# hobincar/reconstruction-network-for-video-captioning

Measured on NVIDIA B200. Metric: train samples/s (decoder+local rec fwd+bwd), higher is better.
Workload: dtype bf16

## Files before the change

reconstruction-network-for-video-captioning_b200/csrc/seq_decoder_cluster.cuh:

```cuda
#pragma once
#include <stdio.h>

#include "proj_attn.cuh"

namespace dcl {
constexpr int CS = 16;
constexpr int THREADS = 512;
constexpr int NWARP = THREADS / 32;
constexpr int MAX_MS = 16;
constexpr int MT = 16;
constexpr int H_ = 512, A_ = 128, UPC = 32, APC = 8, NR = APC + 4 * UPC;
constexpr int NRP = 144;
constexpr int PITCH = H_ + 8;
constexpr int MAXF = 2;
constexpr int MAXT = 32;

__device__ __forceinline__ uint32_t cta_rank() { uint32_t r; asm volatile("mov.u32 %0, %%cluster_ctarank;" : "=r"(r)); return r; }
__device__ __forceinline__ uint32_t cluster_id() { uint32_t r; asm volatile("mov.u32 %0, %%clusterid.x;" : "=r"(r)); return r; }
__device__ __forceinline__ void cluster_barrier() {
  asm volatile("barrier.cluster.arrive.release.aligned;" ::: "memory");
  asm volatile("barrier.cluster.wait.acquire.aligned;" ::: "memory");
}
__device__ __forceinline__ void cluster_arrive() { asm volatile("barrier.cluster.arrive.release.aligned;" ::: "memory"); }
__device__ __forceinline__ void cluster_wait() { asm volatile("barrier.cluster.wait.acquire.aligned;" ::: "memory"); }
__device__ __forceinline__ uint32_t smem_addr(const void* p) { return (uint32_t)__cvta_generic_to_shared(p); }
__device__ __forceinline__ uint32_t mapa(uint32_t saddr, uint32_t rank) {
  uint32_t r;
  asm volatile("mapa.shared::cluster.u32 %0, %1, %2;" : "=r"(r) : "r"(saddr), "r"(rank));
  return r;
}
__device__ __forceinline__ void st_c_f32(uint32_t a, float v) { asm volatile("st.shared::cluster.f32 [%0], %1;" ::"r"(a), "f"(v) : "memory"); }
__device__ __forceinline__ void st_c_f32x2(uint32_t a, float x, float y) { asm volatile("st.shared::cluster.v2.f32 [%0], {%1, %2};" ::"r"(a), "f"(x), "f"(y) : "memory"); }
__device__ __forceinline__ void st_c_f32x4(uint32_t a, float4 v) {
  asm volatile("st.shared::cluster.v4.f32 [%0], {%1, %2, %3, %4};" ::"r"(a), "f"(v.x), "f"(v.y), "f"(v.z), "f"(v.w) : "memory");
}
__device__ __forceinline__ void st_c_u32x4(uint32_t a, uint4 v) {
  asm volatile("st.shared::cluster.v4.b32 [%0], {%1, %2, %3, %4};" ::"r"(a), "r"(v.x), "r"(v.y), "r"(v.z), "r"(v.w) : "memory");
}
__device__ __forceinline__ void stamp(int tag) {
  if (g_timeline != nullptr && blockIdx.x == 0 && threadIdx.x == 0) {
    unsigned long long t;
    asm volatile("mov.u64 %0, %%globaltimer;" : "=l"(t));
    const unsigned int i = atomicAdd(&g_timeline_n, 1u);
    if (i < 4000) g_timeline[i] = (t & 0x00FFFFFFFFFFFFFFull) | ((unsigned long long)tag << 56);
  }
}
__device__ __forceinline__ void ldsm_x4(uint32_t (&r)[4], uint32_t addr) {
  asm volatile("ldmatrix.sync.aligned.m8n8.x4.shared.b16 {%0, %1, %2, %3}, [%4];" : "=r"(r[0]), "=r"(r[1]), "=r"(r[2]), "=r"(r[3]) : "r"(addr));
}
__device__ __forceinline__ void ldsm_x2(uint32_t (&r)[2], uint32_t addr) {
  asm volatile("ldmatrix.sync.aligned.m8n8.x2.shared.b16 {%0, %1}, [%2];" : "=r"(r[0]), "=r"(r[1]) : "r"(addr));
}
__device__ __forceinline__ void ldsm_x2_t(uint32_t (&r)[2], uint32_t addr) {
  asm volatile("ldmatrix.sync.aligned.m8n8.x2.trans.shared.b16 {%0, %1}, [%2];" : "=r"(r[0]), "=r"(r[1]) : "r"(addr));
}
__device__ __forceinline__ void mma16816(float (&c)[4], const uint32_t (&a)[4], const uint32_t (&b)[2]) {
  asm volatile("mma.sync.aligned.m16n8k16.row.col.f32.bf16.bf16.f32 {%0, %1, %2, %3}, {%4, %5, %6, %7}, {%8, %9}, {%0, %1, %2, %3};"
               : "+f"(c[0]), "+f"(c[1]), "+f"(c[2]), "+f"(c[3])
               : "r"(a[0]), "r"(a[1]), "r"(a[2]), "r"(a[3]), "r"(b[0]), "r"(b[1]));
}

__device__ __forceinline__ int wcat_row(int lr, int r) {
  return lr < APC ? r * APC + lr : A_ + ((lr - APC) / UPC) * H_ + r * UPC + (lr - APC) % UPC;
}

struct FwdArgs {
  const bf16* Wcat;
  const float* Uv;
  const float* attn_w;
  const bf16* VW;
  const float* Gx;
  const float* b_hh;
  float* c;
  float* hiddens;
  bf16* Hop;
  float* Wh; float* e;
  bf16* gates;
  int B, L, Tn, MS;
  float inv_T;
};

struct SmemF { int Ws, hs, og, whs, uvs, es, hst, part, total; };
__host__ __device__ inline SmemF smem_fwd() {
  SmemF s;
  s.Ws = 0;
  s.hs = s.Ws + NR * PITCH * 2;
  s.og = s.hs + MT * PITCH * 2;
  s.whs = s.og + MT * NR * 4;
  s.uvs = s.whs + MT * A_ * 4;
  s.es = s.uvs + MAXF * MT * A_ * 4;
  s.hst = s.es + MT * MAXT * 4;
  s.part = s.hst + NWARP * 32 * 2;
  s.total = s.part + NWARP * MT * APC * 4 + 16;
  return s;
}

template <int NQ, bool SM>
__global__ void __launch_bounds__(THREADS, 1) decoder_fwd_cluster_kernel(const FwdArgs a) {
  extern __shared__ __align__(16) unsigned char smem[];
  const SmemF S = smem_fwd();
  bf16* Ws = reinterpret_cast<bf16*>(smem + S.Ws);
  bf16* hs = reinterpret_cast<bf16*>(smem + S.hs);
  float* og = reinterpret_cast<float*>(smem + S.og);
  float* whs = reinterpret_cast<float*>(smem + S.whs);
  float* uvs = reinterpret_cast<float*>(smem + S.uvs);
  float* es = reinterpret_cast<float*>(smem + S.es);
  bf16* hst = reinterpret_cast<bf16*>(smem + S.hst);
  float* part = reinterpret_cast<float*>(smem + S.part);
  const int r = (int)cta_rank(), q = (int)cluster_id();
  const int tid = threadIdx.x, lane = tid & 31, warp = tid >> 5;
  const int B = a.B, Tn = a.Tn;
  const int b0 = q * a.MS, nb = min(a.MS, B - b0);
  if (nb <= 0) return;

  for (int i = tid; i < NR * (H_ / 8); i += THREADS) {
    const int lr = i / (H_ / 8), c8 = i - lr * (H_ / 8);
    *reinterpret_cast<uint4*>(Ws + (size_t)lr * PITCH + 8 * c8) = *reinterpret_cast<const uint4*>(a.Wcat + (size_t)wcat_row(lr, r) * H_ + 8 * c8);
  }
  for (int i = tid; i < MT * PITCH / 2; i += THREADS) reinterpret_cast<uint32_t*>(hs)[i] = 0u;
  for (int i = tid; i < MAXF * MT * (A_ / 4); i += THREADS) {
    const int f = i / (MT * (A_ / 4)), rem = i - f * (MT * (A_ / 4)), s = rem / (A_ / 4), c4 = rem - s * (A_ / 4);
    const int tau = r + CS * f;
    float4 v = make_float4(0.f, 0.f, 0.f, 0.f);
    if (tau < Tn && s < nb) v = reinterpret_cast<const float4*>(a.Uv + ((size_t)(b0 + s) * Tn + tau) * A_)[c4];
    reinterpret_cast<float4*>(uvs)[i] = v;
  }
  for (int i = tid; i < MT * MAXT; i += THREADS) es[i] = 0.f;
  for (int i = tid; i < MT * A_; i += THREADS) whs[i] = 0.f;
  for (int i = tid; i < MT * NR; i += THREADS) og[i] = 0.f;
  const bool act = warp < nb;
  const int s_w = min(warp, nb - 1), b = b0 + s_w;
  const int j = r * UPC + lane;
  pf::Quad<bf16> v[NQ];
  {
    const bf16* vw = a.VW + ((size_t)b * Tn * H_ + j) * 4;
#pragma unroll
    for (int k = 0; k < NQ; ++k) v[k].load(vw + (size_t)min(k, Tn - 1) * 4 * H_);
  }
  float bh[4];
#pragma unroll
  for (int g = 0; g < 4; ++g) bh[g] = a.b_hh[g * H_ + j];
  const float4 aw4 = reinterpret_cast<const float4*>(a.attn_w)[lane];
  float cstate = 0.f;
  __syncthreads();
  cluster_barrier();

  const uint32_t whs_sa = smem_addr(whs), es_sa = smem_addr(es), hs_sa = smem_addr(hs);
  const int gid = lane >> 2, tig = lane & 3;
  for (int t = 0; t < a.L; ++t) {
    float gx[4];
    {
      const float* gp = a.Gx + ((size_t)t * B + b) * 4 * H_ + j;
#pragma unroll
      for (int g = 0; g < 4; ++g) gx[g] = gp[g * H_];
    }
    stamp(20);
    if (t > 0) {
      cluster_wait();
      const uint32_t a_addr = hs_sa + (uint32_t)(((lane & 15) * PITCH + (lane >> 4) * 8) * 2);
      const uint32_t w_addr = smem_addr(Ws) + (uint32_t)(((lane & 7) * PITCH + ((lane >> 3) & 1) * 8) * 2);
      {
        float acc[4] = {0.f, 0.f, 0.f, 0.f};
#pragma unroll
        for (int kk = 0; kk < 2; ++kk) {
          uint32_t af[4], bfr[2];
          ldsm_x4(af, a_addr + (32 * warp + 16 * kk) * 2);
          ldsm_x2(bfr, w_addr + (32 * warp + 16 * kk) * 2);
          mma16816(acc, af, bfr);
        }
        float* pw = part + warp * (MT * APC);
        *reinterpret_cast<float2*>(pw + gid * APC + 2 * tig) = make_float2(acc[0], acc[1]);
        *reinterpret_cast<float2*>(pw + (gid + 8) * APC + 2 * tig) = make_float2(acc[2], acc[3]);
      }
      __syncthreads();
      {
        const int item = tid & 127, grp = tid >> 7, s_ = item >> 3, c_ = item & 7;
        float sum = 0.f;
#pragma unroll
        for (int w2 = 0; w2 < NWARP; ++w2) sum += part[w2 * (MT * APC) + item];
        const uint32_t dst_off = whs_sa + (uint32_t)((s_ * A_ + r * APC + c_) * 4);
#pragma unroll
        for (int i = 0; i < 4; ++i) st_c_f32(mapa(dst_off, (uint32_t)(grp * 4 + i)), sum);
      }
      stamp(27);
      cluster_arrive();
      {
        float acc0[4] = {0.f, 0.f, 0.f, 0.f}, acc1[4] = {0.f, 0.f, 0.f, 0.f};
        const uint32_t b_addr = w_addr + (uint32_t)((APC + warp * 8) * PITCH * 2);
#pragma unroll 2
        for (int k0 = 0; k0 < H_; k0 += 32) {
          uint32_t af[4], bfr[2], af2[4], bfr2[2];
          ldsm_x4(af, a_addr + k0 * 2);
          ldsm_x2(bfr, b_addr + k0 * 2);
          ldsm_x4(af2, a_addr + (k0 + 16) * 2);
          ldsm_x2(bfr2, b_addr + (k0 + 16) * 2);
          mma16816(acc0, af, bfr);
          mma16816(acc1, af2, bfr2);
        }
        const int n = APC + warp * 8 + 2 * tig;
        *reinterpret_cast<float2*>(og + gid * NR + n) = make_float2(acc0[0] + acc1[0], acc0[1] + acc1[1]);
        *reinterpret_cast<float2*>(og + (gid + 8) * NR + n) = make_float2(acc0[2] + acc1[2], acc0[3] + acc1[3]);
      }
      stamp(21);
      cluster_wait();
      stamp(22);
    }
    {
      const float4 wh = reinterpret_cast<const float4*>(whs + s_w * A_)[lane];
      if (r == 0 && act) reinterpret_cast<float4*>(a.Wh + ((size_t)t * B + b) * A_)[lane] = wh;
      float sc[MAXF];
#pragma unroll
      for (int f = 0; f < MAXF; ++f) {
        const float4 u = reinterpret_cast<const float4*>(uvs + (f * MT + s_w) * A_)[lane];
        float s = aw4.x * act_tanh<true>(wh.x + u.x);
        s = fmaf(aw4.y, act_tanh<true>(wh.y + u.y), s);
        s = fmaf(aw4.z, act_tanh<true>(wh.z + u.z), s);
        sc[f] = fmaf(aw4.w, act_tanh<true>(wh.w + u.w), s);
      }
#pragma unroll
      for (int o = 16; o > 0; o >>= 1)
#pragma unroll
        for (int f = 0; f < MAXF; ++f) sc[f] += __shfl_xor_sync(0xffffffffu, sc[f], o);
      const int f = lane & 1, tau = r + CS * f;
      const float val = f ? sc[1] : sc[0];
      if (act && tau < Tn) {
        st_c_f32(mapa(es_sa + (uint32_t)((s_w * MAXT + tau) * 4), (uint32_t)(lane >> 1)), val);
        if (!SM && lane < 2) a.e[((size_t)t * B + b) * Tn + tau] = val;
      }
    }
    stamp(23);
    cluster_barrier();
    stamp(24);
    if constexpr (SM) {
      float* er = es + s_w * MAXT;
      const float al = warp_softmax<true>(er[lane], lane < Tn);
      __syncwarp();
      if (act) {
        if (lane < Tn) er[lane] = al;
        if (r == 0 && lane < Tn) a.e[((size_t)t * B + b) * Tn + lane] = al;
      }
      __syncwarp();
    }
    {
      float acc[4] = {0.f, 0.f, 0.f, 0.f};
      const float4* e4 = reinterpret_cast<const float4*>(es + s_w * MAXT);
#pragma unroll
      for (int k4 = 0; k4 < NQ / 4; ++k4) {
        const float4 e = e4[k4];
        const float ev[4] = {e.x, e.y, e.z, e.w};
#pragma unroll
        for (int kk = 0; kk < 4; ++kk) {
          float f[4];
          v[4 * k4 + kk].get(f);
#pragma unroll
          for (int g = 0; g < 4; ++g) acc[g] = fmaf(ev[kk], f[g], acc[g]);
        }
      }
      float pre[4];
#pragma unroll
      for (int g = 0; g < 4; ++g) pre[g] = gx[g] + bh[g] + og[s_w * NR + APC + g * UPC + lane] + acc[g] * a.inv_T;
      const float gi = act_sigmoid<true>(pre[0]), gf = act_sigmoid<true>(pre[1]), gt = act_tanh<true>(pre[2]), go = act_sigmoid<true>(pre[3]);
      const float cn = fmaf(gf, cstate, gi * gt);
      const float hn = go * act_tanh<true>(cn);
      const bf16 hb = __float2bfloat16_rn(hn);
      hst[warp * 32 + lane] = hb;
      __syncwarp();
      if (act) {
#pragma unroll
        for (int i = 0; i < 2; ++i) {
          const int item = lane * 2 + i, dst = item >> 2, chunk = item & 3;
          const uint4 val = *reinterpret_cast<const uint4*>(hst + warp * 32 + chunk * 8);
          st_c_u32x4(mapa(hs_sa + (uint32_t)((s_w * PITCH + r * UPC + chunk * 8) * 2), (uint32_t)dst), val);
        }
      }
      cluster_arrive();
      if (act) {
        cstate = cn;
        const size_t o1 = ((size_t)t * B + b) * H_ + j;
        a.c[o1 + (size_t)B * H_] = cn;
        a.hiddens[o1] = hn;
        a.Hop[o1 + (size_t)B * H_] = hb;
        pf::Quad<bf16>::store(a.gates + o1 * 4, gi, gf, gt, go);
      }
    }
    stamp(25);
  }
  cluster_wait();
}

static inline bool cluster_enabled() {
  static const int v = rn_env_int("RECNET_DEC_CLUSTER", 1);
  return v != 0;
}
static inline bool cluster_ok(int B, int Tn, int A, int H) {
  return cluster_enabled() && H == H_ && A == A_ && Tn >= 1 && Tn <= MAXT && B >= 1 && B <= 8 * MAX_MS;
}

template <typename K>
static int launch_cluster(K kern, size_t smem, int B, cudaStream_t st, const void* args_struct_ptr, bool* configured) {
  (void)args_struct_ptr;
  if (!*configured) {
    if (cudaFuncSetAttribute(kern, cudaFuncAttributeNonPortableClusterSizeAllowed, 1) != cudaSuccess) { cudaGetLastError(); return RECNET_ERR_UNSUPPORTED; }
    if (cudaFuncSetAttribute(kern, cudaFuncAttributeMaxDynamicSharedMemorySize, (int)smem) != cudaSuccess) { cudaGetLastError(); return RECNET_ERR_UNSUPPORTED; }
    *configured = true;
  }
  return 0;
}

template <typename K>
static int pick_ms(K kern, size_t smem, int B) {
  cudaLaunchConfig_t cfg = {};
  cfg.gridDim = dim3(8 * CS, 1, 1);
  cfg.blockDim = dim3(THREADS, 1, 1);
  cfg.dynamicSmemBytes = smem;
  cudaLaunchAttribute at[1];
  at[0].id = cudaLaunchAttributeClusterDimension;
  at[0].val.clusterDim.x = CS; at[0].val.clusterDim.y = 1; at[0].val.clusterDim.z = 1;
  cfg.attrs = at; cfg.numAttrs = 1;
  int n = 0;
  if (cudaOccupancyMaxActiveClusters(&n, kern, &cfg) != cudaSuccess) { cudaGetLastError(); return 0; }
  n = rn_env_int("RECNET_DEC_CLUSTERS", n);
  if (rn_env_int("RECNET_DEBUG_CLUSTERS", 0)) fprintf(stderr, "[recnet] decoder cluster kernel: max active %d-CTA clusters = %d\n", CS, n);
  if (n < 1) return 0;
  const int ms = (B + n - 1) / n;
  return ms <= MAX_MS ? ms : 0;
}

template <int NQ, bool SM>
static int launch_fwd_nq(FwdArgs a, cudaStream_t st) {
  auto kern = decoder_fwd_cluster_kernel<NQ, SM>;
  const size_t smem = smem_fwd().total;
  static bool configured = false;
  static int ms_cache_B = -1, ms_cache = 0;
  RN_TRY(launch_cluster(kern, smem, a.B, st, nullptr, &configured));
  if (ms_cache_B != a.B) { ms_cache = pick_ms(kern, smem, a.B); ms_cache_B = a.B; }
  if (ms_cache <= 0) return RECNET_ERR_UNSUPPORTED;
  a.MS = ms_cache;
  const int ncl = (a.B + a.MS - 1) / a.MS;
  cudaLaunchConfig_t cfg = {};
  cfg.gridDim = dim3(ncl * CS, 1, 1);
  cfg.blockDim = dim3(THREADS, 1, 1);
  cfg.dynamicSmemBytes = smem;
  cfg.stream = st;
  cudaLaunchAttribute at[1];
  at[0].id = cudaLaunchAttributeClusterDimension;
  at[0].val.clusterDim.x = CS; at[0].val.clusterDim.y = 1; at[0].val.clusterDim.z = 1;
  cfg.attrs = at; cfg.numAttrs = 1;
  ProfScope prof(KC_LOOP, a.L, ncl * CS, 2, st);
  RN_CUDA_OK(cudaLaunchKernelEx(&cfg, kern, a));
  RN_LAUNCH_OK();
  return 0;
}
static int launch_fwd(const FwdArgs& a, bool softmax, cudaStream_t st) {
  if (softmax) return a.Tn <= 28 ? launch_fwd_nq<28, true>(a, st) : launch_fwd_nq<32, true>(a, st);
  return a.Tn <= 28 ? launch_fwd_nq<28, false>(a, st) : launch_fwd_nq<32, false>(a, st);
}
}
```

reconstruction-network-for-video-captioning_b200/csrc/seq_decoder_pf.cuh:

```cuda
#pragma once
#include "proj_attn.cuh"
#include "seq_decoder.cuh"
#include "seq_decoder_cluster.cuh"

namespace dec {

template <typename T>
struct PfWs {
  int EMBp, Vp, Vld, NP;
  GemmPlan pl_h, pl_dh;
  T *Wemb, *WctxI, *Wcat, *U, *Wout, *feats;
  float* Uv; T* VW; T* Xe; float* Gx; T* Hop; float* P; float* Wh; float* e; T* gates; float* c;
  float *logits, *lse, *row_loss;
  T* dlogits; float* dHext; T* dGW; float* dhP; float* dWh; float* dUv; T* dUv_op; float* dw_acc; float* dc; float* dXe; T* ctx;
  float* splitk; float* splitk2; float* splitk3; int* err;
  size_t bytes;
};

static inline bool pf_enabled() {
  static const int v = rn_env_int("RECNET_PF", 1);
  return v != 0;
}
static inline bool pf_ok(const recnet_decoder_desc& d) {
  if (!pf_enabled() || d.cell != RECNET_CELL_LSTM || d.n_layers > 1) return false;
  const int al = d.precision == RECNET_PREC_BF16 ? 8 : 4;
  if ((long long)d.B * d.T * 4 * d.H >= (1ll << 31) || (long long)d.L * d.B * (d.A + 4 * d.H) >= (1ll << 31)) return false;
  if ((d.E & 1) || pf::escore_smem(d.L, d.T, true) > 46 * 1024) return false;
  return d.T >= 1 && d.T <= pf::MAX_T && d.A >= 4 && d.A <= pf::MAX_A && d.A % al == 0 && d.H % al == 0 &&
         pf::bwd_smem_bytes(d.H, d.A) <= 46 * 1024;
}
enum class DecPath { ML, PF, GENERAL };
static inline DecPath dec_path(const recnet_decoder_desc& d) {
  if (d.n_layers > 1) return DecPath::ML;
  return pf_ok(d) ? DecPath::PF : DecPath::GENERAL;
}

template <typename T>
static PfWs<T> plan_pf(const recnet_decoder_desc& d, void* base) {
  PfWs<T> w;
  const int B = d.B, L = d.L, H = d.H, E = d.E, A = d.A, V = d.V, Tn = d.T;
  w.EMBp = round_up(d.EMB, Prec<T>::kpad);
  w.Vp = round_up(V, 8);
  w.Vld = round_up(V, 4);
  w.NP = A + 4 * H;
  w.pl_h = plan_gemm<T>(B, w.NP, H);
  w.pl_dh = plan_gemm<T>(B, H, w.NP);
  if (Prec<T>::id == RECNET_PREC_BF16) {
    w.pl_h.bn = 64;
    const int tiles = rn_cdiv(B, tc::BM) * rn_cdiv(w.NP, 64), nkb = rn_cdiv(H, tc::BK);
    int sp = NUM_SMS / tiles; if (sp < 1) sp = 1; if (sp > nkb) sp = nkb;
    w.pl_h.splits = rn_cdiv(nkb, rn_cdiv(nkb, sp));
    const int nkb2 = rn_cdiv(w.NP, tc::BK);
    if (w.pl_dh.splits > pf::MAXS) w.pl_dh.splits = rn_cdiv(nkb2, rn_cdiv(nkb2, pf::MAXS));
    static const int eh = rn_env_int("RECNET_PF_SPLITS_H", 0);
    static const int edh = rn_env_int("RECNET_PF_SPLITS_DH", 0);
    static const int ebn = rn_env_int("RECNET_PF_BN_H", 0);
    if (ebn == 64 || ebn == 128) w.pl_h.bn = ebn;
    if (eh > 0) w.pl_h.splits = rn_cdiv(nkb, rn_cdiv(nkb, eh > nkb ? nkb : eh));
    if (edh > 0) w.pl_dh.splits = rn_cdiv(nkb2, rn_cdiv(nkb2, edh > nkb2 ? nkb2 : edh));
  }
  Bump m(base);
  w.Wemb = m.take<T>((size_t)4 * H * w.EMBp);
  w.WctxI = m.take<T>((size_t)4 * H * E);
  w.Wcat = m.take<T>((size_t)w.NP * H);
  w.U = m.take<T>((size_t)A * E);
  w.Wout = m.take<T>((size_t)V * H);
  w.feats = m.take<T>((size_t)B * Tn * E);
  w.Uv = m.take<float>((size_t)B * Tn * A);
  w.VW = m.take<T>((size_t)B * Tn * 4 * H);
  w.Xe = m.take<T>((size_t)L * B * w.EMBp);
  w.Gx = m.take<float>((size_t)L * B * 4 * H);
  w.Hop = m.take<T>((size_t)(L + 1) * B * H);
  w.P = m.take<float>((size_t)w.pl_h.splits * B * w.NP);
  w.Wh = m.take<float>((size_t)L * B * A);
  w.e = m.take<float>((size_t)L * B * Tn);
  w.gates = m.take<T>((size_t)L * B * 4 * H);
  w.c = m.take<float>((size_t)(L + 1) * B * H);
  w.logits = m.take<float>((size_t)L * B * w.Vld);
  w.lse = m.take<float>((size_t)L * B);
  w.row_loss = m.take<float>((size_t)L * B);
  w.dlogits = m.take<T>((size_t)L * B * w.Vp);
  w.dHext = m.take<float>((size_t)L * B * H);
  w.dGW = m.take<T>((size_t)L * B * w.NP);
  w.dhP = m.take<float>((size_t)w.pl_dh.splits * B * H);
  w.dWh = m.take<float>((size_t)L * B * A);
  w.dUv = m.take<float>((size_t)B * Tn * A);
  w.dUv_op = m.take<T>((size_t)B * Tn * A);
  w.dw_acc = m.take<float>((size_t)B * A);
  w.dc = m.take<float>((size_t)B * H);
  w.dXe = m.take<float>((size_t)L * B * w.EMBp);
  w.ctx = m.take<T>((size_t)L * B * E);
  w.splitk = m.take<float>(SPLITK_SCRATCH_FLOATS);
  w.splitk2 = m.take<float>(SPLITK_SCRATCH_FLOATS);
  w.splitk3 = m.take<float>(SPLITK_SCRATCH_FLOATS);
  w.err = m.take<int>(64);
  w.bytes = m.off + 256;
  return w;
}

static inline int gemm_to_operand(const float* A, long long lda, const float* B, long long ldb, float* C, long long ldc, int M,
                                  int N, int K, float* scratch, cudaStream_t st) {
  return gemm_full<float>(A, lda, 0, B, ldb, 0, C, ldc, nullptr, M, N, K, 0, scratch, st);
}
static inline int gemm_to_operand(const bf16* A, long long lda, const bf16* B, long long ldb, bf16* C, long long ldc, int M, int N,
                                  int K, float*, cudaStream_t st) {
  GemmPlan p = plan_gemm_full<bf16>(M, N, K);
  if (p.splits > 1) p = plan_gemm<bf16>(M, N, K);
  return tc::launch(A, lda, 0, B, ldb, 0, nullptr, 0, C, ldc, nullptr, M, N, K, 1, 0, 0, p.bn, st);
}

template <typename T>
static int forward_pf(const DecDesc& d, const recnet_decoder_tensors& p, const float* feats, const long long* tokens_in,
                      const long long* targets, const float* ce_weight, const unsigned long long* rng, void* ws, long long ws_bytes,
                      float* hiddens, float* ce_out, cudaStream_t st, int phases = 3) {
  RN_TRY(check(d));
  PfWs<T> w = plan_pf<T>(d, ws);
  if ((long long)w.bytes > ws_bytes) return RECNET_ERR_WORKSPACE;
  const int B = d.B, L = d.L, H = d.H, E = d.E, A = d.A, V = d.V, Tn = d.T, EMB = d.EMB;
  const float p_emb = d.train ? d.p_emb_drop : 0.f, p_out = d.train ? d.p_out_drop : 0.f;
  const float inv_T = d.softmax ? 1.f : 1.f / Tn;
  const long long ldih = EMB + E;
  if (phases & 1) {
  cudaStream_t s2;
  RN_TRY(side().fork(st, &s2));
  misc::embed_gather_kernel<T><<<L * B, 128, 0, s2>>>(p.embedding, tokens_in, w.Xe, w.EMBp, L * B, EMB, w.EMBp, V, d.embedding_scale,
                                                      p_emb, rng, SITE_EMB);
  RN_LAUNCH_OK();
  misc::Stager<T> sg;
  sg.add(feats, E, w.feats, E, (long long)B * Tn, E, E);
  sg.add(p.attn_U, E, w.U, E, A, E, E);
  sg.add(p.w_ih, ldih, w.Wemb, w.EMBp, 4 * H, EMB, w.EMBp);
  sg.add(p.w_ih + EMB, ldih, w.WctxI, E, 4 * H, E, E, H);
  sg.add(p.attn_W, H, w.Wcat, H, A, H, H);
  sg.add(p.w_hh, H, w.Wcat + (size_t)A * H, H, 4 * H, H, H);
  sg.add(p.out_w, H, w.Wout, H, V, H, H);
  sg.zero(w.Hop, (size_t)B * H * sizeof(T));
  sg.zero(w.c, (size_t)B * H * sizeof(float));
  sg.zero(w.err, 64 * sizeof(int));
  RN_TRY(sg.launch(st));
  RN_TRY(side().fork(st, &s2));
  RN_TRY(gemm_full<T>(w.feats, E, 0, w.U, E, 0, w.Uv, A, p.attn_b, B * Tn, A, E, 0, w.splitk2, s2));
  RN_TRY(gemm_full<T>(w.Xe, w.EMBp, 0, w.Wemb, w.EMBp, 0, w.Gx, 4 * H, p.b_ih, L * B, 4 * H, w.EMBp, 0, w.splitk2, s2));
  RN_TRY(gemm_to_operand(w.feats, E, w.WctxI, E, w.VW, 4 * H, B * Tn, 4 * H, E, w.splitk, st));
  RN_TRY(side().join(st, s2));
  bool clustered = false;
  if constexpr (std::is_same<T, bf16>::value) {
    if (dcl::cluster_ok(B, Tn, A, H)) {
      dcl::FwdArgs ca{};
      ca.Wcat = w.Wcat; ca.Uv = w.Uv; ca.attn_w = p.attn_w; ca.VW = w.VW; ca.Gx = w.Gx; ca.b_hh = p.b_hh; ca.c = w.c; ca.hiddens = hiddens;
      ca.Hop = w.Hop; ca.Wh = w.Wh; ca.e = w.e; ca.gates = w.gates; ca.B = B; ca.L = L; ca.Tn = Tn; ca.inv_T = inv_T;
      const int rc = dcl::launch_fwd(ca, d.softmax, st);
      if (rc == 0) clustered = true;
      else if (rc != RECNET_ERR_UNSUPPORTED) return rc;
    }
  }
  for (int t = 0; t < L && !clustered; ++t) {
    const size_t r = (size_t)t * B;
    if (t > 0)
      RN_TRY(gemm_partials<T>(w.Hop + r * H, H, 0, w.Wcat, H, 0, w.P, B, w.NP, H, w.pl_h, st));
    pf::FwdArgs fa{};
    fa.P = w.P; fa.n_p = t > 0 ? w.pl_h.splits : 0; fa.p_stride = (long long)B * w.NP; fa.NP = w.NP;
    fa.Uv = w.Uv; fa.attn_w = p.attn_w; fa.VW = w.VW;
    fa.Gx = w.Gx + r * 4 * H; fa.b_hh = p.b_hh; fa.c_prev = w.c + r * H;
    fa.B = B; fa.Tn = Tn; fa.A = A; fa.H = H; fa.inv_T = inv_T;
    fa.Wh_out = w.Wh + r * A; fa.e_out = w.e + r * Tn; fa.gates_out = w.gates + r * 4 * H;
    fa.c_out = w.c + (r + B) * H; fa.h_out = hiddens + r * H; fa.h_op = w.Hop + (r + B) * H;
    RN_TRY((pf::launch_fwd<T, T>(fa, d.softmax, st)));
  }
  }
  if (!(phases & 2)) return 0;
  const bool training = targets && ce_weight && ce_out;
  cudaStream_t s3 = st;
  if (training) RN_TRY(side().fork(st, &s3));
  RN_TRY(gemm_full<T>(w.Hop + (size_t)B * H, H, 0, w.Wout, H, 0, w.logits, w.Vld, p.out_b, L * B, V, H, 0, w.splitk, st));
  if (training) {
    const int spc = 1;
    pf::pf_escore_kernel<T, true><<<dim3(rn_cdiv(E, 512), rn_cdiv(B, spc)), 256, pf::escore_smem(L, Tn, true), s3>>>(w.e, w.feats, E, 0, w.ctx, L, B,
                                                                                                               Tn, E, inv_T, spc);
    RN_LAUNCH_OK();
  }
  if (targets && ce_weight && ce_out) {
    ProfScope prof(KC_CE, L * B, V, 0, st);
    loss::ce_fwd_kernel<<<L * B, loss::CE_THREADS, 0, st>>>(w.logits, w.Vld, targets, ce_weight, V, p_out, rng, SITE_LOGITS, w.lse,
                                                            w.row_loss);
    RN_LAUNCH_OK();
    loss::sum_kernel<<<1, 1024, 0, st>>>(w.row_loss, L * B, ce_out, 1.f);
    RN_LAUNCH_OK();
  }
  if (training) RN_TRY(side().join(st, s3));
  return 0;
}

template <typename T>
static int backward_pf(const DecDesc& d, const recnet_decoder_tensors& p, const float* feats, const long long* tokens_in,
                       const long long* targets, const float* ce_weight, const unsigned long long* rng, void* ws, long long ws_bytes,
                       const float* g_ce, const float* g_hiddens, const recnet_decoder_tensors& g, cudaStream_t st, int phases = 15) {
  RN_TRY(check(d));
  PfWs<T> w = plan_pf<T>(d, ws);
  if ((long long)w.bytes > ws_bytes) return RECNET_ERR_WORKSPACE;
  const int B = d.B, L = d.L, H = d.H, E = d.E, A = d.A, V = d.V, Tn = d.T, EMB = d.EMB;
  const float p_emb = d.train ? d.p_emb_drop : 0.f, p_out = d.train ? d.p_out_drop : 0.f;
  const int LB = L * B, NP = w.NP;
  const T* Hall = w.Hop + (size_t)B * H;
  if (phases & 1) {
    {
      ProfScope prof(KC_CE, LB, V, 1, st);
      loss::ce_bwd_kernel<T><<<LB, loss::CE_THREADS, 0, st>>>(w.logits, w.Vld, targets, ce_weight, w.lse, g_ce, V, w.Vp, p_out, rng,
                                                              SITE_LOGITS, w.dlogits, w.Vp);
    }
    RN_LAUNCH_OK();
    RN_TRY(gemm_full<T>(w.dlogits, w.Vp, 0, w.Wout, H, 1, w.dHext, H, nullptr, LB, H, V, 0, w.splitk, st));
  }
  for (int t = L - 1; t >= 0 && (phases & 2); --t) {
    const bool last = (t == L - 1);
    const size_t r = (size_t)t * B;
    pf::BwdArgs ba{};
    ba.dh_ext = w.dHext + r * H; ba.dh_ext2 = g_hiddens ? g_hiddens + r * H : nullptr;
    ba.dhP = last ? nullptr : w.dhP; ba.n_p = w.pl_dh.splits; ba.p_stride = (long long)B * H;
    ba.dc = w.dc; ba.first = last ? 1 : 0;
    ba.gates = w.gates + r * 4 * H; ba.c_prev = w.c + r * H; ba.c_new = w.c + (r + B) * H;
    ba.VW = w.VW; ba.Wh = w.Wh + r * A; ba.Uv = w.Uv; ba.attn_w = p.attn_w;
    ba.B = B; ba.Tn = Tn; ba.A = A; ba.H = H; ba.inv_T = d.softmax ? 1.f : 1.f / Tn; ba.alpha = d.softmax ? w.e + r * Tn : nullptr;
    ba.dGW = w.dGW + r * NP; ba.dgw_ld = NP; ba.dWh_out = w.dWh + r * A;
    ba.dUv_acc = w.dUv; ba.uv_first = last ? 1 : 0; ba.dw_acc = w.dw_acc; ba.dw_first = last ? 1 : 0;
    RN_TRY((pf::launch_bwd<T, T>(ba, st)));
    if (t > 0) RN_TRY(gemm_partials<T>(w.dGW + r * NP, NP, 0, w.Wcat, H, 1, w.dhP, B, H, NP, w.pl_dh, st));
  }
  const long long ldih = EMB + E;
  const T* dG = w.dGW + A;
  if (phases == 4) {
    RN_TRY(gemm_full<T>(w.dlogits, w.Vp, 1, Hall, H, 1, g.out_w, H, nullptr, V, H, LB, 0, w.splitk3, st));
    return 0;
  }
  if (!(phases & 8)) return 0;
  cudaStream_t s2;
  RN_TRY(side().fork(st, &s2));
  if (phases & 4) RN_TRY(gemm_full<T>(w.dlogits, w.Vp, 1, Hall, H, 1, g.out_w, H, nullptr, V, H, LB, 0, w.splitk2, s2));
  RN_TRY(misc::colsum<T>(w.dlogits, w.Vp, LB, V, g.out_b, 0, w.splitk2, s2));
  RN_TRY(gemm_full<T>(dG, NP, 1, w.Xe, w.EMBp, 1, g.w_ih, ldih, nullptr, 4 * H, EMB, LB, 0, w.splitk2, s2));
  RN_TRY(gemm_full<T>(dG, NP, 0, w.Wemb, w.EMBp, 1, w.dXe, w.EMBp, nullptr, LB, EMB, 4 * H, 0, w.splitk2, s2));
  RN_CUDA_OK(cudaMemsetAsync(g.embedding, 0, (size_t)V * EMB * sizeof(float), s2));
  misc::embed_scatter_kernel<<<LB, 128, 0, s2>>>(g.embedding, tokens_in, w.dXe, w.EMBp, LB, EMB, V, d.embedding_scale, p_emb, rng,
                                                 SITE_EMB);
  RN_LAUNCH_OK();
  RN_TRY(gemm_full<T>(w.dGW, NP, 1, w.Hop, H, 1, g.attn_W, H, nullptr, A, H, LB, 0, w.splitk2, s2));
  RN_TRY(misc::colsum<T>(dG, NP, LB, 4 * H, g.b_ih, 0, w.splitk, st, g.b_hh));
  RN_TRY(gemm_full<T>(dG, NP, 1, w.ctx, E, 1, g.w_ih + EMB, ldih, nullptr, 4 * H, E, LB, 0, w.splitk, st));
  RN_TRY(gemm_full<T>(dG, NP, 1, w.Hop, H, 1, g.w_hh, H, nullptr, 4 * H, H, LB, 0, w.splitk, st));
  RN_TRY(misc::cast_pad<T>(w.dUv, A, w.dUv_op, A, (long long)B * Tn, A, A, st));
  RN_TRY(gemm_full<T>(w.dUv_op, A, 1, w.feats, E, 1, g.attn_U, E, nullptr, A, E, B * Tn, 0, w.splitk, st));
  RN_TRY(misc::colsum<float>(w.dWh, A, LB, A, g.attn_b, 0, w.splitk, st));
  RN_TRY(misc::colsum<float>(w.dw_acc, A, B, A, g.attn_w, 0, w.splitk, st));
  RN_TRY(side().join(st, s2));
  return 0;
}
template <typename T>
struct GreedyPfWs {
  int EMBp, Vld, NP;
  GemmPlan pl_h;
  T *Wemb, *WctxI, *Wcat, *U, *Wout, *feats, *Emb;
  float* Uv; T* VW; float* EW; T* Hop; float* P; float* c; float* hid; float* logits; long long* tok; int* nonpad; float* splitk;
  size_t bytes;
};
template <typename T>
static GreedyPfWs<T> plan_greedy_pf(const recnet_decoder_desc& d, void* base, int max_steps) {
  GreedyPfWs<T> w;
  const int B = d.B, H = d.H, E = d.E, A = d.A, V = d.V, Tn = d.T;
  w.EMBp = round_up(d.EMB, Prec<T>::kpad);
  w.Vld = round_up(V, 4);
  w.NP = A + 4 * H;
  w.pl_h = plan_gemm<T>(B, w.NP, H);
  Bump m(base);
  w.Wemb = m.take<T>((size_t)4 * H * w.EMBp);
  w.WctxI = m.take<T>((size_t)4 * H * E);
  w.Wcat = m.take<T>((size_t)w.NP * H);
  w.U = m.take<T>((size_t)A * E);
  w.Wout = m.take<T>((size_t)V * H);
  w.feats = m.take<T>((size_t)B * Tn * E);
  w.Emb = m.take<T>((size_t)V * w.EMBp);
  w.Uv = m.take<float>((size_t)B * Tn * A);
  w.VW = m.take<T>((size_t)B * Tn * 4 * H);
  w.EW = m.take<float>((size_t)V * 4 * H);
  w.Hop = m.take<T>((size_t)2 * B * H);
  w.P = m.take<float>((size_t)w.pl_h.splits * B * w.NP);
  w.c = m.take<float>((size_t)2 * B * H);
  w.hid = m.take<float>((size_t)B * H);
  w.logits = m.take<float>((size_t)B * w.Vld);
  w.tok = m.take<long long>(B);
  w.nonpad = m.take<int>(max_steps);
  w.splitk = m.take<float>(SPLITK_SCRATCH_FLOATS);
  w.bytes = m.off + 256;
  return w;
}
static inline bool greedy_pf_ok(const recnet_decoder_desc& d) {
  static const int on = rn_env_int("RECNET_GREEDY_PF", 1);
  return on && d.precision == RECNET_PREC_BF16 && pf_ok(d) && (long long)d.V * 4 * d.H < (1ll << 31);
}

static int greedy_pf(const DecDesc& d0, const recnet_decoder_tensors& p, const float* feats, int max_steps, void* ws,
                     long long ws_bytes, long long* ids_out, int* n_steps_out, cudaStream_t st) {
  typedef bf16 T;
  DecDesc d = d0; d.L = 1; d.train = 0;
  RN_TRY(check(d));
  GreedyPfWs<T> w = plan_greedy_pf<T>(d, ws, max_steps);
  if ((long long)w.bytes > ws_bytes) return RECNET_ERR_WORKSPACE;
  const int B = d.B, H = d.H, E = d.E, A = d.A, V = d.V, Tn = d.T, EMB = d.EMB;
  const long long ldih = EMB + E;
  misc::Stager<T> sg;
  sg.add(feats, E, w.feats, E, (long long)B * Tn, E, E);
  sg.add(p.attn_U, E, w.U, E, A, E, E);
  sg.add(p.w_ih, ldih, w.Wemb, w.EMBp, 4 * H, EMB, w.EMBp);
  sg.add(p.w_ih + EMB, ldih, w.WctxI, E, 4 * H, E, E, H);
  sg.add(p.attn_W, H, w.Wcat, H, A, H, H);
  sg.add(p.w_hh, H, w.Wcat + (size_t)A * H, H, 4 * H, H, H);
  sg.add(p.out_w, H, w.Wout, H, V, H, H);
  sg.add(p.embedding, EMB, w.Emb, w.EMBp, V, EMB, w.EMBp);
  sg.zero(w.Hop, (size_t)2 * B * H * sizeof(T));
  sg.zero(w.c, (size_t)2 * B * H * sizeof(float));
  sg.zero(w.nonpad, (size_t)max_steps * sizeof(int));
  RN_TRY(sg.launch(st));
  RN_TRY(gemm_full<T>(w.feats, E, 0, w.U, E, 0, w.Uv, A, p.attn_b, B * Tn, A, E, 0, w.splitk, st));
  RN_TRY(gemm_to_operand(w.feats, E, w.WctxI, E, w.VW, 4 * H, B * Tn, 4 * H, E, w.splitk, st));
  RN_TRY(gemm_full<T>(w.Emb, w.EMBp, 0, w.Wemb, w.EMBp, 0, w.EW, 4 * H, nullptr, V, 4 * H, w.EMBp, 0, w.splitk, st));
  misc::scale_add_bias_kernel<<<NUM_SMS * 4, 256, 0, st>>>(w.EW, (long long)V * 4 * H, 4 * H, d.embedding_scale, p.b_ih);
  RN_LAUNCH_OK();
  fill_tokens_kernel<<<rn_cdiv(B, 128), 128, 0, st>>>(w.tok, B, 1 );
  RN_LAUNCH_OK();
  for (int t = 0; t < max_steps; ++t) {
    T* h_p = w.Hop + (size_t)(t & 1) * B * H;
    T* h_n = w.Hop + (size_t)((t + 1) & 1) * B * H;
    float* c_p = w.c + (size_t)(t & 1) * B * H;
    float* c_n = w.c + (size_t)((t + 1) & 1) * B * H;
    if (t > 0) RN_TRY(gemm_partials<T>(h_p, H, 0, w.Wcat, H, 0, w.P, B, w.NP, H, w.pl_h, st));
    pf::FwdArgs fa{};
    fa.P = w.P; fa.n_p = t > 0 ? w.pl_h.splits : 0; fa.p_stride = (long long)B * w.NP; fa.NP = w.NP;
    fa.Uv = w.Uv; fa.attn_w = p.attn_w; fa.VW = w.VW;
    fa.Gx = w.EW; fa.gx_rows = w.tok; fa.b_hh = p.b_hh; fa.c_prev = c_p;
    fa.B = B; fa.Tn = Tn; fa.A = A; fa.H = H; fa.inv_T = d.softmax ? 1.f : 1.f / Tn;
    fa.Wh_out = nullptr; fa.e_out = nullptr; fa.gates_out = nullptr;
    fa.c_out = c_n; fa.h_out = w.hid; fa.h_op = h_n;
    RN_TRY((pf::launch_fwd<T, T>(fa, d.softmax, st)));
    RN_TRY(gemm_full<T>(h_n, H, 0, w.Wout, H, 0, w.logits, w.Vld, p.out_b, B, V, H, 0, w.splitk, st));
    argmax_feedback_kernel<<<B, 256, 0, st>>>(w.logits, w.Vld, V, ids_out + (size_t)t * B, w.tok, w.nonpad + t);
    RN_LAUNCH_OK();
  }
  greedy_finalize_kernel<<<1, 1, 0, st>>>(w.nonpad, max_steps, n_steps_out);
  RN_LAUNCH_OK();
  return 0;
}
}
```

Baseline: 48240.

## Add persistent cluster kernel for decoder LSTM backward time loop

Adds a thread-block-cluster persistent kernel that runs the whole decoder backward recurrence over time steps in one launch. It keeps recurrent weights in shared memory and exchanges dh and attention partial sums through distributed shared memory with cluster barriers. This replaces the per-timestep launch of the pf backward kernel plus a split-K GEMM. The cost is a complex synchronisation scheme, and it falls back to the old path when the shape is unsupported.

```diff
diff --git a/reconstruction-network-for-video-captioning_b200/csrc/seq_decoder_cluster.cuh b/reconstruction-network-for-video-captioning_b200/csrc/seq_decoder_cluster.cuh
--- a/reconstruction-network-for-video-captioning_b200/csrc/seq_decoder_cluster.cuh
+++ b/reconstruction-network-for-video-captioning_b200/csrc/seq_decoder_cluster.cuh
@@ -288,6 +288,286 @@
   cluster_wait();
 }
 
+struct BwdArgs {
+  const bf16* Wcat;
+  const float* Uv;
+  const float* attn_w;
+  const bf16* VW;
+  const bf16* gates;
+  const float* c;
+  const float* Wh;
+  const float* alpha;
+  const float* dHext;
+  const float* g_hiddens;
+  bf16* dGW;
+  float* dWh;
+  float* dUv;
+  float* dw_acc;
+  int B, L, Tn, MS;
+  float inv_T;
+};
+
+constexpr int XP = NRP + 8;
+struct SmemB { int Ws, xs, dhr, uvs, der, dwr, sad, total; };
+__host__ __device__ inline SmemB smem_bwd() {
+  SmemB s;
+  s.Ws = 0;
+  s.xs = s.Ws + NRP * PITCH * 2;
+  s.dhr = s.xs + MT * XP * 2;
+  s.uvs = s.dhr + CS * MT * UPC * 4;
+  s.der = s.uvs + MAXF * MT * A_ * 4;
+  s.dwr = s.der + CS * MT * MAXF * 4;
+  s.sad = s.dwr + CS * MT * APC * 4;
+  s.total = s.sad + CS * MT * 4 + 16;
+  return s;
+}
+
+__device__ __forceinline__ void stamp_cluster_entry(int q) {
+  if (g_timeline != nullptr && cta_rank() == 0 && threadIdx.x == 0 && q < 8) {
+    unsigned long long t;
+    asm volatile("mov.u64 %0, %%globaltimer;" : "=l"(t));
+    const unsigned int i = atomicAdd(&g_timeline_n, 1u);
+    if (i < 4000) g_timeline[i] = (t & 0x00FFFFFFFFFFFFFFull) | ((unsigned long long)(48 + q) << 56);
+  }
+}
+
+__device__ __forceinline__ void quad_get_in_loop(const pf::Quad<bf16>& q, float (&f)[4]) {
+  pf::Quad<bf16> c;
+  asm volatile("mov.b32 %0, %1;" : "=r"(c.r.x) : "r"(q.r.x));
+  asm volatile("mov.b32 %0, %1;" : "=r"(c.r.y) : "r"(q.r.y));
+  c.get(f);
+}
+
+template <int NQ, bool SM>
+__global__ void __launch_bounds__(THREADS, 1) decoder_bwd_cluster_kernel(const BwdArgs a) {
+  extern __shared__ __align__(16) unsigned char smem[];
+  const SmemB S = smem_bwd();
+  bf16* Ws = reinterpret_cast<bf16*>(smem + S.Ws);
+  bf16* xs = reinterpret_cast<bf16*>(smem + S.xs);
+  float* dhr = reinterpret_cast<float*>(smem + S.dhr);
+  float* uvs = reinterpret_cast<float*>(smem + S.uvs);
+  float* der = reinterpret_cast<float*>(smem + S.der);
+  float* dwr = reinterpret_cast<float*>(smem + S.dwr);
+  float* sad = reinterpret_cast<float*>(smem + S.sad);
+  const int r = (int)cta_rank(), q = (int)cluster_id();
+  const int tid = threadIdx.x, lane = tid & 31, warp = tid >> 5;
+  const int B = a.B, Tn = a.Tn;
+  constexpr int NP = A_ + 4 * H_;
+  const int b0 = q * a.MS, nb = min(a.MS, B - b0);
+  if (nb <= 0) return;
+  stamp_cluster_entry(q);
+
+  for (int i = tid; i < NRP * (H_ / 8); i += THREADS) {
+    const int lr = i / (H_ / 8), c8 = i - lr * (H_ / 8);
+    uint4 w = make_uint4(0u, 0u, 0u, 0u);
+    if (lr < NR) w = *reinterpret_cast<const uint4*>(a.Wcat + (size_t)wcat_row(lr, r) * H_ + 8 * c8);
+    *reinterpret_cast<uint4*>(Ws + (size_t)lr * PITCH + 8 * c8) = w;
+  }
+  for (int i = tid; i < MT * XP / 2; i += THREADS) reinterpret_cast<uint32_t*>(xs)[i] = 0u;
+  for (int i = tid; i < MAXF * MT * (A_ / 4); i += THREADS) {
+    const int f = i / (MT * (A_ / 4)), rem = i - f * (MT * (A_ / 4)), s = rem / (A_ / 4), c4 = rem - s * (A_ / 4);
+    const int tau = r + CS * f;
+    float4 v = make_float4(0.f, 0.f, 0.f, 0.f);
+    if (tau < Tn && s < nb) v = reinterpret_cast<const float4*>(a.Uv + ((size_t)(b0 + s) * Tn + tau) * A_)[c4];
+    reinterpret_cast<float4*>(uvs)[i] = v;
+  }
+  const bool act = warp < nb;
+  const int s_w = min(warp, nb - 1), b = b0 + s_w;
+  const int j = r * UPC + lane;
+  pf::Quad<bf16> v[NQ];
+  {
+    const bf16* vw = a.VW + ((size_t)b * Tn * H_ + j) * 4;
+#pragma unroll
+    for (int k = 0; k < NQ; ++k) v[k].load(vw + (size_t)min(k, Tn - 1) * 4 * H_);
+  }
+  const float4 aw4 = reinterpret_cast<const float4*>(a.attn_w)[lane];
+  float dcar = 0.f;
+  float4 duv[MAXF], dwv = make_float4(0.f, 0.f, 0.f, 0.f);
+#pragma unroll
+  for (int f = 0; f < MAXF; ++f) duv[f] = make_float4(0.f, 0.f, 0.f, 0.f);
+  __syncthreads();
+  cluster_barrier();
+
+  const uint32_t dhr_sa = smem_addr(dhr), der_sa = smem_addr(der), dwr_sa = smem_addr(dwr), sad_sa = smem_addr(sad);
+  const int gid = lane >> 2, tig = lane & 3;
+  const uint32_t a_addr = smem_addr(xs) + (uint32_t)(((lane & 15) * XP + (lane >> 4) * 8) * 2);
+  const uint32_t b_addr = smem_addr(Ws) + (uint32_t)(((lane & 15) * PITCH + 32 * warp) * 2);
+  for (int t = a.L - 1; t >= 0; --t) {
+    const size_t row = (size_t)t * B + b;
+    pf::Quad<bf16> gq;
+    gq.load(a.gates + (row * H_ + j) * 4);
+    const float cp = a.c[row * H_ + j], cn = a.c[(row + B) * H_ + j];
+    float dh = a.dHext[row * H_ + j];
+    const float dhe2 = a.g_hiddens ? a.g_hiddens[row * H_ + j] : 0.f;
+    const float4 wh = reinterpret_cast<const float4*>(a.Wh + row * A_)[lane];
+    float al[MAXF];
+    if constexpr (SM) {
+#pragma unroll
+      for (int f = 0; f < MAXF; ++f) al[f] = r + CS * f < Tn ? a.alpha[row * Tn + r + CS * f] : 0.f;
+    }
+    stamp(30);
+    dh += dhe2;
+    if (t < a.L - 1) {
+      cluster_wait();
+#pragma unroll
+      for (int src = 0; src < CS; ++src) dh += dhr[(src * MT + s_w) * UPC + lane];
+    }
+    float dg[4];
+    {
+      float g[4];
+      gq.get(g);
+      const float tc = act_tanh<true>(cn);
+      const float dc = fmaf(dh * g[3], 1.f - tc * tc, dcar);
+      const bf16 r0 = __float2bfloat16_rn(dc * g[2] * g[0] * (1.f - g[0]));
+      const bf16 r1 = __float2bfloat16_rn(dc * cp * g[1] * (1.f - g[1]));
+      const bf16 r2 = __float2bfloat16_rn(dc * g[0] * (1.f - g[2] * g[2]));
+      const bf16 r3 = __float2bfloat16_rn(dh * tc * g[3] * (1.f - g[3]));
+      dcar = dc * g[1];
+      if (act) {
+        bf16* o = a.dGW + row * NP + A_ + j;
+        o[0] = r0; o[H_] = r1; o[2 * H_] = r2; o[3 * H_] = r3;
+        bf16* x = xs + s_w * XP + APC + lane;
+        x[0] = r0; x[UPC] = r1; x[2 * UPC] = r2; x[3 * UPC] = r3;
+      }
+      dg[0] = __bfloat162float(r0); dg[1] = __bfloat162float(r1); dg[2] = __bfloat162float(r2); dg[3] = __bfloat162float(r3);
+    }
+    {
+      float p[16];
+      const bool upper = (lane & 16) != 0;
+#pragma unroll
+      for (int k = 0; k < 16; ++k) {
+        float x[4];
+        quad_get_in_loop(v[k], x);
+        const float lo = fmaf(dg[0], x[0], fmaf(dg[1], x[1], fmaf(dg[2], x[2], dg[3] * x[3])));
+        float hi = 0.f;
+        if (k + 16 < NQ) {
+          quad_get_in_loop(v[k + 16], x);
+          hi = fmaf(dg[0], x[0], fmaf(dg[1], x[1], fmaf(dg[2], x[2], dg[3] * x[3])));
+        }
+        p[k] = (upper ? hi : lo) + __shfl_xor_sync(0xffffffffu, upper ? lo : hi, 16);
+      }
+#pragma unroll
+      for (int s = 8; s >= 1; s >>= 1) {
+        const bool up = (lane & s) != 0;
+#pragma unroll
+        for (int i = 0; i < s; ++i) {
+          const float send = up ? p[i] : p[i + s];
+          const float keep = up ? p[i + s] : p[i];
+          p[i] = keep + __shfl_xor_sync(0xffffffffu, send, s);
+        }
+      }
+      const float de_part = p[0];
+      if (act && lane < Tn) st_c_f32(mapa(der_sa + (uint32_t)(((r * MT + s_w) * MAXF + (lane >> 4)) * 4), (uint32_t)(lane & 15)), de_part);
+    }
+    __syncthreads();
+    stamp(31);
+    cluster_arrive();
+    float acc[4][4];
+#pragma unroll
+    for (int n = 0; n < 4; ++n) acc[n][0] = acc[n][1] = acc[n][2] = acc[n][3] = 0.f;
+    if (t > 0) {
+#pragma unroll
+      for (int kt = 1; kt < NRP / 16; ++kt) {
+        uint32_t af[4];
+        ldsm_x4(af, a_addr + kt * 16 * 2);
+#pragma unroll
+        for (int n = 0; n < 4; ++n) {
+          uint32_t bfr[2];
+          ldsm_x2_t(bfr, b_addr + (uint32_t)((kt * 16 * PITCH + 8 * n) * 2));
+          mma16816(acc[n], af, bfr);
+        }
+      }
+    }
+    stamp(32);
+    cluster_wait();
+    stamp(33);
+    {
+      float de[MAXF];
+#pragma unroll
+      for (int f = 0; f < MAXF; ++f) {
+        float s = 0.f;
+#pragma unroll
+        for (int src = 0; src < CS; ++src) s += der[(src * MT + s_w) * MAXF + f];
+        de[f] = r + CS * f < Tn ? s * a.inv_T : 0.f;
+      }
+      if constexpr (SM) {
+        const float sa = fmaf(al[1], de[1], al[0] * de[0]);
+        if (act && lane < CS) st_c_f32(mapa(sad_sa + (uint32_t)((r * MT + s_w) * 4), (uint32_t)lane), sa);
+        cluster_barrier();
+        float tot = 0.f;
+#pragma unroll
+        for (int src = 0; src < CS; ++src) tot += sad[src * MT + s_w];
+#pragma unroll
+        for (int f = 0; f < MAXF; ++f) de[f] = al[f] * (de[f] - tot);
+      }
+      float4 dwh = make_float4(0.f, 0.f, 0.f, 0.f);
+#pragma unroll
+      for (int f = 0; f < MAXF; ++f) {
+        if (r + CS * f < Tn) {
+          const float g = de[f];
+          const float4 u = reinterpret_cast<const float4*>(uvs + (f * MT + s_w) * A_)[lane];
+          const float tx = act_tanh<true>(wh.x + u.x), ty = act_tanh<true>(wh.y + u.y);
+          const float tz = act_tanh<true>(wh.z + u.z), tw = act_tanh<true>(wh.w + u.w);
+          const float4 ds = make_float4(g * aw4.x * (1.f - tx * tx), g * aw4.y * (1.f - ty * ty), g * aw4.z * (1.f - tz * tz),
+                                        g * aw4.w * (1.f - tw * tw));
+          dwh = pf::f4_add(dwh, ds);
+          duv[f] = pf::f4_add(duv[f], ds);
+          dwv = pf::f4_add(dwv, make_float4(g * tx, g * ty, g * tz, g * tw));
+        }
+      }
+      if (act) st_c_f32x4(mapa(dwr_sa + (uint32_t)(((r * MT + s_w) * APC + (lane & 1) * 4) * 4), (uint32_t)(lane >> 1)), dwh);
+    }
+    stamp(34);
+    cluster_barrier();
+    if (tid < MT * APC) {
+      const int s_ = tid >> 3, c_ = tid & 7;
+      float sum = 0.f;
+#pragma unroll
+      for (int src = 0; src < CS; ++src) sum += dwr[(src * MT + s_) * APC + c_];
+      if (s_ < nb) {
+        const size_t orow = (size_t)t * B + b0 + s_;
+        const bf16 hb = __float2bfloat16_rn(sum);
+        a.dWh[orow * A_ + r * APC + c_] = sum;
+        a.dGW[orow * NP + r * APC + c_] = hb;
+        xs[s_ * XP + c_] = hb;
+      }
+    }
+    if (t > 0) {
+      __syncthreads();
+#pragma unroll
+      for (int n = 0; n < 4; ++n) {
+        uint32_t af[4], bfr[2];
+        ldsm_x4(af, a_addr);
+        ldsm_x2_t(bfr, b_addr + (uint32_t)(8 * n * 2));
+        mma16816(acc[n], af, bfr);
+      }
+      const uint32_t dst = dhr_sa + (uint32_t)((r * MT * UPC + gid * UPC + 2 * tig) * 4);
+#pragma unroll
+      for (int n = 0; n < 4; ++n) {
+        st_c_f32x2(mapa(dst + 8 * n * 4, (uint32_t)warp), acc[n][0], acc[n][1]);
+        st_c_f32x2(mapa(dst + (8 * UPC + 8 * n) * 4, (uint32_t)warp), acc[n][2], acc[n][3]);
+      }
+      stamp(35);
+      cluster_arrive();
+    }
+  }
+  if (act) {
+#pragma unroll
+    for (int f = 0; f < MAXF; ++f)
+      if (r + CS * f < Tn) reinterpret_cast<float4*>(a.dUv + ((size_t)b * Tn + r + CS * f) * A_)[lane] = duv[f];
+    st_c_f32x4(mapa(dhr_sa + (uint32_t)(((r * MT + s_w) * APC + (lane & 1) * 4) * 4), (uint32_t)(lane >> 1)), dwv);
+  }
+  cluster_barrier();
+  if (tid < MT * APC) {
+    const int s_ = tid >> 3, c_ = tid & 7;
+    float sum = 0.f;
+#pragma unroll
+    for (int src = 0; src < CS; ++src) sum += dhr[(src * MT + s_) * APC + c_];
+    if (s_ < nb) a.dw_acc[(size_t)(b0 + s_) * A_ + r * APC + c_] = sum;
+  }
+  stamp(36);
+}
+
 static inline bool cluster_enabled() {
   static const int v = rn_env_int("RECNET_DEC_CLUSTER", 1);
   return v != 0;
@@ -326,16 +606,13 @@
   return ms <= MAX_MS ? ms : 0;
 }
 
-template <int NQ, bool SM>
-static int launch_fwd_nq(FwdArgs a, cudaStream_t st) {
-  auto kern = decoder_fwd_cluster_kernel<NQ, SM>;
-  const size_t smem = smem_fwd().total;
-  static bool configured = false;
-  static int ms_cache_B = -1, ms_cache = 0;
-  RN_TRY(launch_cluster(kern, smem, a.B, st, nullptr, &configured));
-  if (ms_cache_B != a.B) { ms_cache = pick_ms(kern, smem, a.B); ms_cache_B = a.B; }
-  if (ms_cache <= 0) return RECNET_ERR_UNSUPPORTED;
-  a.MS = ms_cache;
+template <typename Args>
+static int launch_loop(void (*kern)(Args), size_t smem, Args a, int prof_steps, bool* configured, int* ms_cache_B, int* ms_cache,
+                       cudaStream_t st) {
+  RN_TRY(launch_cluster(kern, smem, a.B, st, nullptr, configured));
+  if (*ms_cache_B != a.B) { *ms_cache = pick_ms(kern, smem, a.B); *ms_cache_B = a.B; }
+  if (*ms_cache <= 0) return RECNET_ERR_UNSUPPORTED;
+  a.MS = *ms_cache;
   const int ncl = (a.B + a.MS - 1) / a.MS;
   cudaLaunchConfig_t cfg = {};
   cfg.gridDim = dim3(ncl * CS, 1, 1);
@@ -346,13 +623,34 @@
   at[0].id = cudaLaunchAttributeClusterDimension;
   at[0].val.clusterDim.x = CS; at[0].val.clusterDim.y = 1; at[0].val.clusterDim.z = 1;
   cfg.attrs = at; cfg.numAttrs = 1;
-  ProfScope prof(KC_LOOP, a.L, ncl * CS, 2, st);
+  ProfScope prof(KC_LOOP, prof_steps, ncl * CS, 2, st);
   RN_CUDA_OK(cudaLaunchKernelEx(&cfg, kern, a));
   RN_LAUNCH_OK();
   return 0;
 }
+template <int NQ, bool SM>
+static int launch_fwd_nq(const FwdArgs& a, cudaStream_t st) {
+  static bool configured = false;
+  static int ms_cache_B = -1, ms_cache = 0;
+  return launch_loop(decoder_fwd_cluster_kernel<NQ, SM>, smem_fwd().total, a, a.L, &configured, &ms_cache_B, &ms_cache, st);
+}
 static int launch_fwd(const FwdArgs& a, bool softmax, cudaStream_t st) {
   if (softmax) return a.Tn <= 28 ? launch_fwd_nq<28, true>(a, st) : launch_fwd_nq<32, true>(a, st);
   return a.Tn <= 28 ? launch_fwd_nq<28, false>(a, st) : launch_fwd_nq<32, false>(a, st);
 }
-}
+
+static inline bool cluster_bwd_enabled() {
+  static const int v = rn_env_int("RECNET_DEC_CLUSTER_BWD", 1);
+  return v != 0;
+}
+template <int NQ, bool SM>
+static int launch_bwd_nq(const BwdArgs& a, cudaStream_t st) {
+  static bool configured = false;
+  static int ms_cache_B = -1, ms_cache = 0;
+  return launch_loop(decoder_bwd_cluster_kernel<NQ, SM>, smem_bwd().total, a, a.L - 1, &configured, &ms_cache_B, &ms_cache, st);
+}
+static int launch_bwd(const BwdArgs& a, bool softmax, cudaStream_t st) {
+  if (softmax) return a.Tn <= 28 ? launch_bwd_nq<28, true>(a, st) : launch_bwd_nq<32, true>(a, st);
+  return a.Tn <= 28 ? launch_bwd_nq<28, false>(a, st) : launch_bwd_nq<32, false>(a, st);
+}
+}
diff --git a/reconstruction-network-for-video-captioning_b200/csrc/seq_decoder_pf.cuh b/reconstruction-network-for-video-captioning_b200/csrc/seq_decoder_pf.cuh
--- a/reconstruction-network-for-video-captioning_b200/csrc/seq_decoder_pf.cuh
+++ b/reconstruction-network-for-video-captioning_b200/csrc/seq_decoder_pf.cuh
@@ -211,7 +211,20 @@
     RN_LAUNCH_OK();
     RN_TRY(gemm_full<T>(w.dlogits, w.Vp, 0, w.Wout, H, 1, w.dHext, H, nullptr, LB, H, V, 0, w.splitk, st));
   }
-  for (int t = L - 1; t >= 0 && (phases & 2); --t) {
+  bool clustered = false;
+  if constexpr (std::is_same<T, bf16>::value) {
+    if ((phases & 2) && dcl::cluster_ok(B, Tn, A, H) && dcl::cluster_bwd_enabled()) {
+      dcl::BwdArgs ca{};
+      ca.Wcat = w.Wcat; ca.Uv = w.Uv; ca.attn_w = p.attn_w; ca.VW = w.VW; ca.gates = w.gates; ca.c = w.c; ca.Wh = w.Wh;
+      ca.alpha = d.softmax ? w.e : nullptr; ca.dHext = w.dHext; ca.g_hiddens = g_hiddens;
+      ca.dGW = w.dGW; ca.dWh = w.dWh; ca.dUv = w.dUv; ca.dw_acc = w.dw_acc;
+      ca.B = B; ca.L = L; ca.Tn = Tn; ca.inv_T = d.softmax ? 1.f : 1.f / Tn;
+      const int rc = dcl::launch_bwd(ca, d.softmax, st);
+      if (rc == 0) clustered = true;
+      else if (rc != RECNET_ERR_UNSUPPORTED) return rc;
+    }
+  }
+  for (int t = L - 1; t >= 0 && (phases & 2) && !clustered; --t) {
     const bool last = (t == L - 1);
     const size_t r = (size_t)t * B;
     pf::BwdArgs ba{};
```

After: 48320 (median of 6 runs). About the same (+0.2%).
